# Christina-hshi/SH-assembly

Hardware: AMD Instinct MI355X
Metric: k-mers counted/sec (whole node), CQF build, C.elegans-like k=47 (higher is better)
Workload: dtype u64

## Files before the change

### sh-assembly_amd/csrc/partition_kernels.hip

```cpp
#include "shk_device.h"

#define SHK_RP_TILE 4096
#define SHK_RP_MAXP 1024
#define SHK_SCAN_TILE 2048

struct ShkRpLevel {
  uint32_t shift;
  uint32_t bits;
  uint32_t nbuckets;
  uint32_t hb;
  uint64_t q_lo;
  uint64_t nslots;
  uint32_t out32;
  uint32_t ablate;
  uint32_t slot_cap;
  uint32_t ng_log2;
};

__device__ __forceinline__ uint32_t shk_word_region(uint64_t w, uint32_t hb, uint64_t q_lo) {
  uint64_t key = hb >= 64 ? w : (w & ((1ULL << hb) - 1));
  return (uint32_t)(((key >> 8) - q_lo) >> SHK_REGION_LOG2);
}

template <typename T>
__global__ void k_scan_reduce(const T *in, uint64_t n_host, const uint64_t *n_dev, uint64_t *block_sums) {
  __shared__ uint64_t scratch[SHK_MAX_WAVES + 1];
  const uint64_t n = n_dev ? *n_dev : n_host;
  const uint64_t base = (uint64_t)blockIdx.x * SHK_SCAN_TILE;
  uint64_t s = 0;
  for (uint64_t i = base + threadIdx.x; i < base + SHK_SCAN_TILE && i < n; i += blockDim.x) s += in[i];
  uint64_t tot = shk_block_sum64(s, scratch);
  if (threadIdx.x == 0) block_sums[blockIdx.x] = tot;
}
__global__ void k_scan_top(uint64_t *block_sums, uint64_t nblocks, uint64_t *total) {
  __shared__ uint64_t scratch[SHK_MAX_WAVES + 1];
  __shared__ uint64_t carry_s;
  if (threadIdx.x == 0) carry_s = 0;
  __syncthreads();
  for (uint64_t b = 0; b < nblocks; b += blockDim.x) {
    uint64_t i = b + threadIdx.x;
    uint64_t v = i < nblocks ? block_sums[i] : 0, tot;
    uint64_t ex = shk_block_exscan64(v, &tot, scratch);
    uint64_t carry = carry_s;
    if (i < nblocks) block_sums[i] = carry + ex;
    __syncthreads();
    if (threadIdx.x == 0) carry_s = carry + tot;
    __syncthreads();
  }
  if (threadIdx.x == 0) *total = carry_s;
}
template <typename T>
__global__ void k_scan_apply(const T *in, uint64_t n_host, const uint64_t *n_dev, const uint64_t *block_sums,
                             const uint64_t *total, uint64_t *out) {
  __shared__ uint64_t scratch[SHK_MAX_WAVES + 1];
  const uint64_t n = n_dev ? *n_dev : n_host;
  const uint64_t base = (uint64_t)blockIdx.x * SHK_SCAN_TILE;
  if (base > n) return;
  const unsigned per = SHK_SCAN_TILE / blockDim.x;
  const uint64_t my = base + (uint64_t)threadIdx.x * per;
  uint64_t s = 0;
  for (unsigned j = 0; j < per; j++)
    if (my + j < n) s += in[my + j];
  uint64_t tot;
  uint64_t ex = shk_block_exscan64(s, &tot, scratch) + block_sums[blockIdx.x];
  for (unsigned j = 0; j < per; j++) {
    if (my + j < n) { out[my + j] = ex; ex += in[my + j]; }
  }
  if (threadIdx.x == 0 && n >= base && n < base + SHK_SCAN_TILE) out[n] = *total;
}

__global__ void k_rp_base1(const uint64_t *n_p, uint64_t *bucket_base) {
  if (threadIdx.x == 0 && blockIdx.x == 0) { bucket_base[0] = 0; bucket_base[1] = *n_p; }
}

__global__ void k_rp_tile_first(const uint64_t *bucket_base, uint32_t nbuckets, const uint64_t *n_p, uint32_t *tfb) {
  const uint64_t n = *n_p;
  const uint64_t w = (uint64_t)blockIdx.x * blockDim.x + threadIdx.x;
  const uint64_t pos = w * SHK_RP_TILE;
  if (pos >= n) return;
  uint32_t lo = 0, hi = nbuckets;
  while (hi - lo > 1) {
    uint32_t mid = (lo + hi) / 2;
    if (bucket_base[mid] <= pos) lo = mid; else hi = mid;
  }
  tfb[w] = lo;
}

__global__ void k_rp_hist(const uint64_t *words, const uint64_t *n_p, const uint64_t *bucket_base,
                          const uint32_t *tfb, ShkRpLevel lv, uint64_t *hist, uint32_t wtiles) {
  __shared__ uint32_t lh[SHK_RP_MAXP];
  const uint64_t n = *n_p;
  const uint64_t wstart = (uint64_t)blockIdx.x * wtiles * SHK_RP_TILE;
  if (wstart >= n) return;
  const uint64_t wend = wstart + (uint64_t)wtiles * SHK_RP_TILE < n ? wstart + (uint64_t)wtiles * SHK_RP_TILE : n;
  const uint32_t P = 1u << lv.bits;
  for (uint32_t b = tfb[(uint64_t)blockIdx.x * wtiles]; b < lv.nbuckets && bucket_base[b] < wend; b++) {
    const uint64_t lo = bucket_base[b] > wstart ? bucket_base[b] : wstart;
    const uint64_t hi = bucket_base[b + 1] < wend ? bucket_base[b + 1] : wend;
    if (hi <= lo) continue;
    for (uint32_t d = threadIdx.x; d < (P << lv.ng_log2); d += blockDim.x) lh[d] = 0;
    __syncthreads();
    for (uint64_t i0 = lo; i0 < hi; i0 += 4ull * blockDim.x) {
      uint64_t w[4];
#pragma unroll
      for (int u = 0; u < 4; u++) {
        const uint64_t i = i0 + (uint64_t)u * blockDim.x + threadIdx.x;
        w[u] = i < hi ? words[i] : 0;
      }
#pragma unroll
      for (int u = 0; u < 4; u++) {
        const uint64_t i = i0 + (uint64_t)u * blockDim.x + threadIdx.x;
        if (i < hi) {
          const uint32_t dg = (shk_word_region(w[u], lv.hb, lv.q_lo) >> lv.shift) & (P - 1);
          const uint32_t grp = (uint32_t)(i >> SHK_RP_TILE0_LOG2) & ((1u << lv.ng_log2) - 1);
          atomicAdd(&lh[(dg << lv.ng_log2) | grp], 1u);
        }
      }
    }
    __syncthreads();
    for (uint32_t d = threadIdx.x; d < (P << lv.ng_log2); d += blockDim.x)
      if (lh[d]) atomicAdd((unsigned long long *)&hist[(((uint64_t)b * P) << lv.ng_log2) + d], (unsigned long long)lh[d]);
    __syncthreads();
  }
}

__global__ void k_rp_group_bases(const uint64_t *sub, uint32_t nd, uint32_t ng_log2, uint64_t *base) {
  const uint32_t d = blockIdx.x * blockDim.x + threadIdx.x;
  if (d <= nd) base[d] = sub[(uint64_t)d << ng_log2];
}

#define SHK_RP_THREADS 512
#define SHK_RP_KPT (SHK_RP_TILE / SHK_RP_THREADS)
template <int LB2>
__global__ void k_rp_hist2(const uint64_t *words, const uint64_t *n_p, ShkRpLevel lv0, ShkRpLevel lv1, uint64_t *hist0, uint64_t *hist1,
                           uint32_t wtiles) {
  __shared__ uint32_t lh0[SHK_RP_MAXP];
  __shared__ uint32_t lh1[1u << LB2];
  const uint64_t n = *n_p;
  const uint64_t wstart = (uint64_t)blockIdx.x * wtiles * SHK_RP_TILE;
  if (wstart >= n) return;
  const uint64_t wend = wstart + (uint64_t)wtiles * SHK_RP_TILE < n ? wstart + (uint64_t)wtiles * SHK_RP_TILE : n;
  const uint32_t P0 = 1u << lv0.bits, C = 1u << (lv0.bits + lv1.bits);
  for (uint32_t d = threadIdx.x; d < (P0 << lv0.ng_log2); d += blockDim.x) lh0[d] = 0;
  for (uint32_t d = threadIdx.x; d < C; d += blockDim.x) lh1[d] = 0;
  __syncthreads();
  for (uint64_t i0 = wstart; i0 < wend; i0 += 4ull * blockDim.x) {
    uint64_t w[4];
#pragma unroll
    for (int u = 0; u < 4; u++) {
      const uint64_t i = i0 + (uint64_t)u * blockDim.x + threadIdx.x;
      w[u] = i < wend ? words[i] : 0;
    }
#pragma unroll
    for (int u = 0; u < 4; u++) {
      const uint64_t i = i0 + (uint64_t)u * blockDim.x + threadIdx.x;
      if (i < wend) {
        const uint32_t region = shk_word_region(w[u], lv0.hb, lv0.q_lo);
        const uint32_t d0 = (region >> lv0.shift) & (P0 - 1);
        const uint32_t grp = (uint32_t)(i >> SHK_RP_TILE0_LOG2) & ((1u << lv0.ng_log2) - 1);
        atomicAdd(&lh0[(d0 << lv0.ng_log2) | grp], 1u);
        atomicAdd(&lh1[(region >> lv1.shift) & (C - 1)], 1u);
      }
    }
  }
  __syncthreads();
  for (uint32_t d = threadIdx.x; d < (P0 << lv0.ng_log2); d += blockDim.x)
    if (lh0[d]) atomicAdd((unsigned long long *)&hist0[d], (unsigned long long)lh0[d]);
  for (uint32_t d = threadIdx.x; d < C; d += blockDim.x)
    if (lh1[d]) atomicAdd((unsigned long long *)&hist1[d], (unsigned long long)lh1[d]);
}

__global__ void k_rp_slot_cursors(uint64_t *cursor, uint64_t n, uint32_t cap) {
  const uint64_t stride = (uint64_t)gridDim.x * blockDim.x;
  for (uint64_t i = (uint64_t)blockIdx.x * blockDim.x + threadIdx.x; i < n; i += stride) cursor[i] = i * cap;
}

template <int TILE_LOG2, int THREADS, int PMAX = SHK_RP_MAXP>
__global__ void __launch_bounds__(THREADS) k_rp_scatter(const uint64_t *in, uint64_t *out, const uint64_t *n_p,
                                                        const uint64_t *bucket_base, const uint32_t *tfb, ShkRpLevel lv,
                                                        uint64_t *cursor, uint32_t *err) {
  constexpr uint32_t SHK_RP_TILE_ = 1u << TILE_LOG2;
  constexpr int KPT_ = (int)(SHK_RP_TILE_ / THREADS);
  static_assert(SHK_RP_TILE_ <= 65536, "a rank inside a digit takes 16 bits");
  __shared__ uint32_t lh[PMAX];
  __shared__ uint32_t lbase[PMAX];
  __shared__ uint64_t gbase[PMAX];
  __shared__ uint64_t stage[SHK_RP_TILE_];
  __shared__ uint32_t scratch[SHK_MAX_WAVES + 1];
  const uint64_t n = *n_p;
  const uint64_t wstart = (uint64_t)blockIdx.x * SHK_RP_TILE_;
  if (wstart >= n) return;
  const uint64_t wend = wstart + SHK_RP_TILE_ < n ? wstart + SHK_RP_TILE_ : n;
  const uint32_t P = 1u << lv.bits;
  for (uint32_t b = (lv.nbuckets > 1 ? tfb[(uint64_t)blockIdx.x << (TILE_LOG2 - 12)] : 0u); b < lv.nbuckets && bucket_base[b] < wend; b++) {
    const uint64_t lo = bucket_base[b] > wstart ? bucket_base[b] : wstart;
    const uint64_t hi = bucket_base[b + 1] < wend ? bucket_base[b + 1] : wend;
    if (hi <= lo) continue;
    const uint32_t cnt = (uint32_t)(hi - lo);
    for (uint32_t d = threadIdx.x; d < P; d += THREADS) lh[d] = 0;
    uint64_t w[KPT_];
#pragma unroll
    for (int u = 0; u < KPT_; u++) {
      const uint32_t i = threadIdx.x + (uint32_t)u * THREADS;
      w[u] = i < cnt ? in[lo + i] : 0;
    }
    __syncthreads();
    uint32_t dr[KPT_];
#pragma unroll
    for (int u = 0; u < KPT_; u++) {
      const uint32_t i = threadIdx.x + (uint32_t)u * THREADS;
      dr[u] = 0;
      if (i < cnt) {
        const uint32_t d = (shk_word_region(w[u], lv.hb, lv.q_lo) >> lv.shift) & (P - 1);
        dr[u] = (d << 16) | atomicAdd(&lh[d], 1u);
      }
    }
    __syncthreads();
    uint32_t carry = 0;
    for (uint32_t d0 = 0; d0 < P; d0 += THREADS) {
      uint32_t d = d0 + threadIdx.x;
      uint32_t v = d < P ? lh[d] : 0, tot;
      uint32_t ex = shk_block_exscan(v, &tot, scratch);
      if (d < P) {
        lbase[d] = carry + ex;
        if (lv.ablate & 1) gbase[d] = cursor[((uint64_t)b * P + d) << lv.ng_log2] + (uint64_t)(blockIdx.x % 1024) * 24;
        else gbase[d] = v ? atomicAdd((unsigned long long *)&cursor[((((uint64_t)b * P) + d) << lv.ng_log2) | (blockIdx.x & ((1u << lv.ng_log2) - 1))], (unsigned long long)v) : 0;
        if (lv.slot_cap && v && gbase[d] + v > ((uint64_t)b * P + d + 1) * lv.slot_cap) {
          atomicOr(err, SHK_E_SLOT_FULL);
          gbase[d] = ~0ULL;
        }
      }
      carry += tot;
    }
    __syncthreads();
#pragma unroll
    for (int u = 0; u < KPT_; u++) {
      const uint32_t i = threadIdx.x + (uint32_t)u * THREADS;
      if (i < cnt) stage[lbase[dr[u] >> 16] + (dr[u] & 0xFFFFu)] = w[u];
    }
    __syncthreads();
    for (uint32_t i = threadIdx.x; i < cnt; i += THREADS) {
      uint64_t x = stage[i];
      uint32_t d = (shk_word_region(x, lv.hb, lv.q_lo) >> lv.shift) & (P - 1);
      if (lv.out32) {
        const uint64_t key = lv.hb >= 64 ? x : (x & ((1ULL << lv.hb) - 1));
        const uint64_t q = (key >> 8) - lv.q_lo;
        if (q >= lv.nslots) atomicOr(err, SHK_E_CORRUPT);
        const uint32_t rec = ((((uint32_t)q & (SHK_REGION - 1)) << 8 | (uint32_t)(key & 0xff)) << SHK_CHUNK_BITS) |
                             ((uint32_t)(x >> lv.hb) & (SHK_MAX_CHUNKS - 1));
        if (gbase[d] != ~0ULL) reinterpret_cast<uint32_t *>(out)[gbase[d] + (i - lbase[d])] = rec;
      } else {
        out[gbase[d] + (i - lbase[d])] = x;
      }
    }
    shk_lds_barrier();
  }
}
```

### sh-assembly_amd/csrc/shk_api.hip

```cpp
#include "../../include/shk.h"
#include <thread>

#include <hip/hip_runtime.h>
#include <math.h>
#include <stdio.h>
#include <stdlib.h>
#include <string.h>
#include <vector>
#include <string>
#include <algorithm>
#include <unordered_set>
#include <unordered_map>

#include "kmer_kernels.hip"
#include "roll_kernels.hip"
#include "partition_kernels.hip"
#include "cqf_kernels.hip"
#include "merge2_kernels.hip"
#include "walk_kernels.hip"
#include "unitig_kernels.hip"

#define SHK_SLACK 256

enum {
  KP_COUNT_LINES, KP_SCAN_CHUNKS, KP_EMIT_READS, KP_COUNT_KEYS, KP_HASH, KP_SCAN, KP_RP_PREP, KP_RP_HIST,
  KP_RP_SCATTER, KP_MERGE_SUM, KP_REGION_SCAN, KP_MERGE_WRITE, KP_MERGE_SPILL, KP_PLACE, KP_MARKS, KP_LOOKUP, KP_WALK, KP_UG_WALK, KP_UG_FINISH, KP_MERGE_FUSED, KP_MERGE_SAMPLE, KP_MISC, KP_ROLL_HIST, KP_ROLL_SCATTER, KP_PACK, KP_RP_SLOTS, KP_N
};
static const char *kp_names[KP_N] = {
  "k_count_lines", "k_scan_chunks", "k_emit_reads", "k_count_keys", "k_hash_reads", "k_scan_*", "k_rp_prep",
  "k_rp_hist", "k_rp_scatter", "k_region_merge<summary>", "k_region_scan", "k_region_merge<write>",
  "k_region_merge<spill>", "k_region_place", "k_denoise_marks", "k_lookup", "k_extend_forward+k_select_seeds", "k_ug_walk", "k_ug_check/emit/median/links", "k_region_merge<fused>", "k_region_merge<sample>", "misc", "k_roll_hist", "k_roll_scatter", "k_pack_reads", "k_rp_slot_cursors"};

struct PendingEvent { int id; hipEvent_t a, b; };

#define SHK_SCALAR_WORDS 64
enum ShkDevSlot {
  DS_NREADS = 0,
  DS_NWORDS = 1,
  DS_SCAN_TOTAL = 2,
  DS_MARKS = 3,
  DS_MAX_COUNT = 4,
  DS_DUMP_STOP = 5,
  DS_WALK_IN = 8,
  DS_WALK_OUT = 10,
  DS_STAMPS = 16,
  DS_PAIR_LEN = 40,
  DS_PAIR_BASE = 42,
  DS_END = 46
};
enum ShkHostSlot {
  HP_COUNTERS = 0,
  HP_ERR = 40,
  HP_NREADS = 41,
  HP_NWORDS = 42,
  HP_NWORDS_IN = 43,
  HP_FREE_PTR = 44,
  HP_TOTAL = 45,
  HP_AUX = 46,
  HP_MARKS = 47,
  HP_IFIN = 48,
  HP_IFIRST = 49,
  HP_WALK_IN = 50,
  HP_WALK_OUT = 52,
  HP_PAIR = 56,
  HP_END = 62
};
enum { CNT_NEWD, CNT_ADDED, CNT_REMOVED, CNT_ADDED_BEFORE };
static_assert(HP_COUNTERS + SHK_NCOUNTERS <= HP_ERR, "the counters mirror ends before the error word");
static_assert(DS_END <= SHK_SCALAR_WORDS && HP_END <= SHK_SCALAR_WORDS, "both blocks fit their 64 words");
static_assert(DS_PAIR_BASE + 4 == DS_END && HP_PAIR + (DS_END - DS_PAIR_LEN) == HP_END, "the pair block is uploaded in one copy");

enum { RP_SCATTER_GROUPED, RP_SCATTER_WIDE, RP_SCATTER_TILE };
struct ShkPartLevel {
  uint8_t scatter;
  bool pair_hist;
  bool may_slot;
};

struct ShkStageBufs {
  hipStream_t stream = hipStream_t();
  bool lent = false;
  uint8_t *d_text = nullptr;
  uint64_t *d_chunk_off = nullptr, *d_chunk_len = nullptr, *d_nlines = nullptr, *d_reads_base = nullptr;
  uint64_t *d_rd_start = nullptr, *d_rd_end = nullptr;
  uint16_t *d_rd_chunk = nullptr;
  uint32_t *d_nkeys = nullptr;
  uint64_t *d_key_base = nullptr;
  uint64_t *d_words[2] = {};
  uint64_t *d_scalars = nullptr;
  uint64_t *d_block_sums = nullptr;
  uint64_t *d_hist[4] = {};
  uint64_t *d_base_sub = nullptr;
  uint64_t *d_base[5] = {};
  uint64_t *d_cursor = nullptr;
  uint32_t *d_tfb = nullptr;
  uint32_t *d_err = nullptr;
  uint64_t *h_pinned = nullptr;
  uint32_t last_err_bits = 0;
  uint32_t region_cap = 0;
  uint32_t slot_overflows = 0;
  int slots_off = 0;
  double prof_ms[KP_N] = {};
  uint64_t prof_n[KP_N] = {};
  std::vector<PendingEvent> pending;
  std::vector<hipEvent_t> evpool;
};

struct shk_ctx : ShkStageBufs {
  shk_config cfg;
// ... 161 lines not shown
  for (uint32_t l = 0; l < 4; l++) hipFree(b->d_hist[l]);
  for (uint32_t l = 0; l < 5; l++) if (!(b->lent && l == c->nlevels)) hipFree(b->d_base[l]);
  hipHostFree(b->h_pinned);
  if (b->stream) hipStreamDestroy(b->stream);
  *b = ShkStageBufs();
}

static int create_init(shk_ctx *c, const shk_config *cfg) {
  const uint32_t ns = cfg->num_shards ? cfg->num_shards : 1;
  c->cfg = *cfg;
  c->dev = cfg->device;
  HIPCHK(hipSetDevice(c->dev));
  c->g_nslots = 1ULL << cfg->qb;
  if (c->g_nslots / ns < 64) return SHK_ERR_ARG;
  c->nslots = c->g_nslots / ns;
  c->q_lo = c->nslots * cfg->shard_index;
  c->xnslots = c->nslots + (uint64_t)(10 * sqrt((double)c->g_nslots));
  c->nblocks = (c->xnslots + 63) / 64;
  c->table_bytes = c->nblocks * SHK_BLOCK_BYTES;
  c->nregions = (uint32_t)((c->nslots + SHK_REGION - 1) / SHK_REGION);
  c->rbits = 0;
  while ((1u << c->rbits) < c->nregions) c->rbits++;
  const uint32_t mlb = cfg->max_level_bits ? cfg->max_level_bits : 10;
  if (mlb > 10) return SHK_ERR_ARG;
  const uint32_t nlevels = (c->rbits + mlb - 1) / mlb;
  if (nlevels > 4) return SHK_ERR_ARG;
  c->nlevels = nlevels ? nlevels : 1;
  {
    uint32_t left = c->rbits, nb = 1;
    for (uint32_t l = 0; l < c->nlevels; l++) {
      uint32_t bits = (left + (c->nlevels - l) - 1) / (c->nlevels - l);
      left -= bits;
      c->lv[l].shift = left; c->lv[l].bits = bits; c->lv[l].nbuckets = nb; c->lv[l].hb = cfg->hb; c->lv[l].q_lo = c->q_lo;
      c->lv[l].nslots = c->nslots; c->lv[l].out32 = 0; c->lv[l].ablate = 0; c->lv[l].ng_log2 = 0; c->lv[l].slot_cap = 0;
      nb <<= bits;
    }
    c->lv[c->nlevels - 1].out32 = 1;
    if (c->lv[0].bits >= 2 && c->lv[0].bits <= 7 && !getenv("SHK_RP_NO_GROUPS")) c->lv[0].ng_log2 = 3;
  }
  c->threads = cfg->threads_per_group ? cfg->threads_per_group : 512;
  if (c->threads < 64 || c->threads > 1024 || (c->threads & (c->threads - 1))) return SHK_ERR_ARG;
  c->hash_groups = cfg->hash_groups ? cfg->hash_groups : 2048;
  c->roll_two = c->nlevels >= 2 && c->lv[0].bits + c->lv[1].bits <= 14;
  for (uint32_t l = 0; l < c->nlevels; l++) {
    const bool last = l + 1 == c->nlevels;
    c->part[l].scatter = l == 0 && c->lv[0].ng_log2 ? RP_SCATTER_GROUPED : c->threads >= 512 && !last && c->lv[l].bits <= 8 ? RP_SCATTER_WIDE : RP_SCATTER_TILE;
    c->part[l].pair_hist = l == 0 && c->roll_two && c->lv[1].ng_log2 == 0;
    c->part[l].may_slot = last && l >= 1 && c->lv[l].out32;
  }
  c->rounds_left = cfg->num_denoise;
  c->max_reads = cfg->max_batch_reads ? cfg->max_batch_reads : cfg->max_batch_bytes / 16 + 1024;
  { int rc = bufs_alloc(c, c, false); if (rc) return rc; }
  for (int i = 0; i < 2; i++) {
    if (dmalloc(&c->tab[i], c->table_bytes)) return SHK_ERR_HIP;
    if (dmalloc(&c->fin[i], (uint64_t)c->nregions + 2)) return SHK_ERR_HIP;
  }
  if (dmalloc(&c->d_summary, SHK_SUM_STRIDE * (uint64_t)c->nregions + 8)) return SHK_ERR_HIP;
  if (dmalloc(&c->d_dump_offs, (uint64_t)c->nregions + 2)) return SHK_ERR_HIP;
  c->sample_stride = c->nregions >= (1u << 20) ? 16 : 8;
  if (const char *e = getenv("SHK_SAMPLE_STRIDE")) c->sample_stride = (uint32_t)atoi(e);
  else if (c->nregions < (1u << 14)) c->sample_stride = 0;
  c->lazy_ok = 1;
  if (const char *e = getenv("SHK_LAZY_PLACE")) c->lazy_ok = atoi(e) != 0;
  if (dmalloc(&c->spill[0], (uint64_t)c->nregions * SHK_SPILL_STRIDE) || dmalloc(&c->d_over_list, (uint64_t)c->nregions + 1)) return SHK_ERR_HIP;
  { uint64_t nt = c->nregions / SHK_RSCAN_TILE + 2;
    if (dmalloc(&c->d_tile_a, nt) || dmalloc(&c->d_tile_b, nt) || dmalloc(&c->d_tile_f, nt)) return SHK_ERR_HIP; }
  if (dmalloc(&c->d_counters, SHK_NCOUNTERS)) return SHK_ERR_HIP;
  HIPCHK(hipMemsetAsync(c->tab[0], 0, c->table_bytes + SHK_SLACK, c->stream));
  HIPCHK(hipMemsetAsync(c->tab[1], 0, c->table_bytes + SHK_SLACK, c->stream));
  HIPCHK(hipMemsetAsync(c->fin[0], 0, ((uint64_t)c->nregions + 2) * 8, c->stream));
  HIPCHK(hipMemsetAsync(c->fin[1], 0, ((uint64_t)c->nregions + 2) * 8, c->stream));
  HIPCHK(hipStreamSynchronize(c->stream));
  if (cfg->num_denoise > 0 || cfg->num_shards > 1) {
    if (ensure_chist(c) || point_alloc(c)) return SHK_ERR_HIP;
  }
  if (cfg->num_shards > 1) {
    for (int b = 0; b < 2; b++)
      if (dmalloc(&c->d_send[b], c->cfg.max_batch_keys + 1)) return SHK_ERR_HIP;
  }
  return SHK_OK;
}
// ... 188 lines not shown
  if (!chunk_labels_ok(nchunks, chunk_first, chunk_mul)) return SHK_ERR_BATCH;
  const uint8_t *dtext;
  uint64_t nreads;
  { int rc = parse_stage(c, b, text, on_device, text_bytes, chunk_off, chunk_len, nchunks, &dtext, &nreads); if (rc) return rc; }
  const uint64_t P = 1ULL << c->lv[0].bits;
  const uint32_t cb = c->lv[0].bits + c->lv[1].bits;
  const bool two = c->roll_two;
  if (two) HIPCHK(hipMemsetAsync(b->d_hist[1], 0, (1ULL << cb) * 8, b->stream));
  else HIPCHK(hipMemsetAsync(b->d_hist[0], 0, P * 8, b->stream));
  ShkRollArgs A;
  roll_args(c, b, A, dtext, text_bytes, chunk_first, chunk_mul);
  A.q_lo = c->q_lo;
  A.dig_shift = c->lv[0].shift; A.dig_bits = c->lv[0].bits;
  A.hist = two ? b->d_hist[1] : b->d_hist[0]; A.hist_shift = two ? c->lv[1].shift : c->lv[0].shift; A.hist_bits = two ? cb : c->lv[0].bits;
  A.cursor = b->d_cursor; A.out = b->d_words[0];
  { int rc = pack_stage(c, b, A, nreads, text_bytes, b->d_words[1]); if (rc) return rc; }
  { ProfScope ps(c, b, KP_ROLL_HIST);
    launch_roll_hist(c, b, A, nreads, two);
    if (two) hipLaunchKernelGGL(k_roll_fold, dim3((uint32_t)(P / 256 + 1)), dim3(256), 0, b->stream, (const uint64_t *)b->d_hist[1], (uint32_t)P,
                                1u << c->lv[1].bits, b->d_hist[0]); }
  if (run_scan<uint64_t>(c, b, b->d_hist[0], P, nullptr, b->d_base[1])) return SHK_ERR_HIP;
  HIPCHK(hipMemcpyAsync(b->d_scalars + DS_NWORDS, b->d_base[1] + P, 8, hipMemcpyDeviceToDevice, b->stream));
  HIPCHK(hipMemcpyAsync(b->d_cursor, b->d_base[1], P * 8, hipMemcpyDeviceToDevice, b->stream));
  launch_roll_scatter(c, b, A, nreads);
  HIPCHK(hipGetLastError());
  return SHK_OK;
}

struct ShkPartInput {
  const uint64_t *src[2]; uint64_t n[2]; int nsrc;
  int in_buf;
  uint32_t first_level;
  bool counted[2];
};
static ShkPartInput part_from_roll(const shk_ctx *c, const ShkStageBufs *b, uint64_t n) { return {{b->d_words[0], nullptr}, {n, 0}, 1, 0, 1, {false, c->roll_two}}; }
static ShkPartInput part_from_hash(const ShkStageBufs *b, uint64_t n) { return {{b->d_words[0], nullptr}, {n, 0}, 1, 0, 0, {true, false}}; }
static ShkPartInput part_from_words(const ShkStageBufs *b, const uint64_t *w, uint64_t n, const uint64_t *w2 = nullptr, uint64_t n2 = 0) {
  return {{w, w2}, {n, n2}, w2 ? 2 : 1, w == b->d_words[0] ? 0 : w == b->d_words[1] ? 1 : -1, 0, {false, false}};
}

static uint32_t slot_capacity(const shk_ctx *c, uint64_t nregions, uint64_t nwords) {
  uint64_t cp = 2 * c->cfg.max_batch_keys / nregions;
  if (cp > (1u << 20)) cp = 1u << 20;
  const double mean = (double)nwords / (double)nregions;
  return cp >= 64 && (double)cp >= mean + 6.0 * sqrt(8.0 * mean + 1.0) + 16.0 ? (uint32_t)cp : 0;
}

static int partition_stage(const shk_ctx *c, ShkStageBufs *b, const ShkPartInput &in, int *dst) {
  const uint64_t *n_p = b->d_scalars + DS_NWORDS;
  const uint64_t nmax = in.n[0] + in.n[1];
  { ProfScope ps(c, b, KP_RP_PREP);
    hipLaunchKernelGGL(k_rp_base1, dim3(1), dim3(64), 0, b->stream, n_p, b->d_base[0]); }
  const uint32_t nwin = (uint32_t)(nmax / SHK_RP_TILE + 1);
  int cur = in.in_buf < 0 ? 1 : in.in_buf;
  bool counted[4] = {in.counted[0], in.counted[1], false, false};
  b->region_cap = 0;
  for (uint32_t l = in.first_level; l < c->nlevels; l++) {
    const ShkPartLevel &pl = c->part[l];
    const uint64_t nb = c->lv[l].nbuckets, P = 1ULL << c->lv[l].bits;
    struct Src { const uint64_t *w, *n_p, *base; uint64_t n; } srcs[2] = {{l == in.first_level ? in.src[0] : b->d_words[cur], n_p, b->d_base[l], nmax}, {}};
    int nsrc = 1;
    if (l == 0 && in.nsrc == 2) {
      srcs[0] = {in.src[0], b->d_scalars + DS_PAIR_LEN, b->d_scalars + DS_PAIR_BASE, in.n[0]};
      srcs[1] = {in.src[1], b->d_scalars + DS_PAIR_LEN + 1, b->d_scalars + DS_PAIR_BASE + 2, in.n[1]};
      nsrc = 2;
    }
    uint32_t cap = pl.may_slot && !b->slots_off && !counted[l] ? slot_capacity(c, nb * P, nmax) : 0;
    { ProfScope ps(c, b, KP_RP_PREP);
      hipLaunchKernelGGL(k_rp_tile_first, dim3(nwin / 256 + 1), dim3(256), 0, b->stream, b->d_base[l], (uint32_t)nb, n_p, b->d_tfb); }
    for (;;) {
      ShkRpLevel lvl = c->lv[l];
#ifdef SHK_DIAGNOSTICS
      if (const char *e = getenv("SHK_RP_ABLATE")) lvl.ablate = (uint32_t)atoi(e);
#endif
      uint64_t *cursor = b->d_cursor;
      if (cap) {
        ProfScope ps(c, b, KP_RP_SLOTS);
        cursor = b->d_base[l + 1];
        lvl.slot_cap = cap;
        hipLaunchKernelGGL(k_rp_slot_cursors, dim3((uint32_t)((nb * P) / 256 + 1 < 4096 ? (nb * P) / 256 + 1 : 4096)), dim3(256), 0, b->stream, cursor, nb * P, cap);
      } else {
        if (!counted[l] && pl.pair_hist) {
          HIPCHK(hipMemsetAsync(b->d_hist[0], 0, (P << c->lv[0].ng_log2) * 8, b->stream));
          HIPCHK(hipMemsetAsync(b->d_hist[1], 0, (P << c->lv[1].bits) * 8, b->stream));
          ProfScope ps(c, b, KP_RP_HIST);
          const uint32_t wt = nwin / 1024 + 1;
          for (int si = 0; si < nsrc; si++)
            hipLaunchKernelGGL((k_rp_hist2<14>), dim3(nwin / wt + 1), dim3(c->threads < 512 ? c->threads : 512), 0, b->stream, srcs[si].w, srcs[si].n_p,
                               c->lv[0], c->lv[1], b->d_hist[0], b->d_hist[1], wt);
          counted[1] = true;
        } else if (!counted[l]) {
          HIPCHK(hipMemsetAsync(b->d_hist[l], 0, ((nb * P) << c->lv[l].ng_log2) * 8, b->stream));
          ProfScope ps(c, b, KP_RP_HIST);
          const uint32_t wt = nwin / 4096 + 1;
          for (int si = 0; si < nsrc; si++)
            hipLaunchKernelGGL(k_rp_hist, dim3(nwin / wt + 1), dim3(c->threads), 0, b->stream, srcs[si].w, srcs[si].n_p, srcs[si].base, b->d_tfb, c->lv[l],
                               b->d_hist[l], wt);
        }
        if (c->lv[l].ng_log2) {
          const uint32_t ng = c->lv[l].ng_log2;
          if (run_scan<uint64_t>(c, b, b->d_hist[l], P << ng, nullptr, b->d_base_sub)) return SHK_ERR_HIP;
          HIPCHK(hipMemcpyAsync(b->d_cursor, b->d_base_sub, (P << ng) * 8, hipMemcpyDeviceToDevice, b->stream));
          ProfScope ps(c, b, KP_RP_PREP);
          hipLaunchKernelGGL(k_rp_group_bases, dim3((uint32_t)(P / 256 + 1)), dim3(256), 0, b->stream, b->d_base_sub, (uint32_t)P, ng, b->d_base[l + 1]);
        } else {
          if (run_scan<uint64_t>(c, b, b->d_hist[l], nb * P, nullptr, b->d_base[l + 1])) return SHK_ERR_HIP;
          HIPCHK(hipMemcpyAsync(b->d_cursor, b->d_base[l + 1], nb * P * 8, hipMemcpyDeviceToDevice, b->stream));
        }
      }
      { ProfScope ps(c, b, KP_RP_SCATTER);
        for (int si = 0; si < nsrc; si++) {
          const Src &S = srcs[si];
          const dim3 wide((uint32_t)(S.n >> SHK_RP_TILE0_LOG2) + 1);
          if (pl.scatter == RP_SCATTER_GROUPED)
            hipLaunchKernelGGL((k_rp_scatter<SHK_RP_TILE0_LOG2, 1024>), wide, dim3(1024), 0, b->stream, S.w, b->d_words[cur ^ 1], S.n_p, S.base,
                               b->d_tfb, lvl, cursor, b->d_err);
          else if (pl.scatter == RP_SCATTER_WIDE)
            hipLaunchKernelGGL((k_rp_scatter<SHK_RP_TILE0_LOG2, 1024, 256>), wide, dim3(1024), 0, b->stream, S.w, b->d_words[cur ^ 1], S.n_p, S.base,
                               b->d_tfb, lvl, cursor, b->d_err);
          else
            hipLaunchKernelGGL((k_rp_scatter<12, SHK_RP_THREADS>), dim3((uint32_t)(S.n / SHK_RP_TILE + 1)), dim3(SHK_RP_THREADS), 0, b->stream, S.w,
                               b->d_words[cur ^ 1], S.n_p, S.base, b->d_tfb, lvl, cursor, b->d_err);
        } }
      if (!cap) break;
      uint32_t bits = 0;
      if (fetch_err(b, &bits)) return SHK_ERR_HIP;
      if (bits & ~SHK_E_SLOT_FULL) return map_err_bits(bits & ~SHK_E_SLOT_FULL);
      if (!bits) { b->region_cap = cap; b->slot_overflows = 0; break; }
      if (++b->slot_overflows >= 2) b->slots_off = 1;
      cap = 0;
    }
    cur ^= 1;
  }
  HIPCHK(hipGetLastError());
  *dst = cur;
  return SHK_OK;
}

#define SHK_REGION_SLICE (1u << 24)
#define SHK_FOR_REGION_SLICES(c, A, nblk) \
  for (uint32_t r0_ = 0, nblk = 0; r0_ < (c)->nregions && ((A).r0 = r0_, nblk = (c)->nregions - r0_ < SHK_REGION_SLICE ? (c)->nregions - r0_ : SHK_REGION_SLICE, true); r0_ += SHK_REGION_SLICE)

template <int MODE>
static void launch_merge(shk_ctx *c, const ShkMergeArgs &A0, bool rec = false) {
  ShkMergeArgs A = A0;
  SHK_FOR_REGION_SLICES(c, A, nblk) {
    if (MODE != 1 && rec)
// ... 550 lines not shown

static int merge_stage(shk_ctx *c, const uint64_t *words, uint32_t nchunks, uint64_t nwords, shk_batch_stats *st) {
  uint32_t lo = 0;
  int rc = merge_stage_from(c, words, nchunks, nwords, st, &lo);
  if (rc == SHK_ERR_REGION && !c->big_image && (c->last_err_bits & (SHK_E_OLD_EXTENT | SHK_E_NEW_EXTENT))) {
    c->big_image = 1;
    c->last_err_bits = 0;
    rc = merge_stage_from(c, words, nchunks, nwords, st, &lo);
  }
  return rc;
}

static int finish(shk_ctx *c, int rc) {
  uint32_t bits = 0;
  int rc2 = fetch_err(c, &bits);
  prof_collect(c);
  if (rc) return rc;
  if (rc2) return rc2;
  return map_err_bits(bits);
}

static int front_end(const shk_ctx *c, ShkStageBufs *b, const void *text, int on_device, uint64_t text_bytes, const uint64_t *chunk_off,
                     const uint64_t *chunk_len, uint32_t nchunks, uint64_t *nwords, int *dst, uint32_t *region_cap) {
  const bool roll = roll_path(c);
  int rc = roll ? roll_stage(c, b, text, on_device, text_bytes, chunk_off, chunk_len, nchunks, 0, 1)
                : hash_stage(c, b, text, on_device, text_bytes, chunk_off, chunk_len, nchunks, 0, 1, true);
  if (rc) return rc;
  uint32_t bits = 0;
  HIPCHK(hipMemcpyAsync(b->h_pinned + HP_NWORDS, b->d_scalars + DS_NWORDS, 8, hipMemcpyDeviceToHost, b->stream));
  if (fetch_err(b, &bits)) return SHK_ERR_HIP;
  if (bits) return map_err_bits(bits);
  *nwords = b->h_pinned[HP_NWORDS];
  if (*nwords > c->cfg.max_batch_keys) return SHK_ERR_BATCH;
  rc = partition_stage(c, b, roll ? part_from_roll(c, b, *nwords) : part_from_hash(b, *nwords), dst);
  *region_cap = b->region_cap;
  return rc;
}

extern "C" int shk_count_chunks(shk_ctx *c, const void *text, int text_on_device, uint64_t text_bytes,
                                const uint64_t *chunk_off, const uint64_t *chunk_len, uint32_t nchunks,
                                shk_batch_stats *stats) {
  if (!c || !text || !chunk_off || !chunk_len) return SHK_ERR_ARG;
  shk_batch_stats st;
  memset(&st, 0, sizeof(st));
  HIPCHK(hipSetDevice(c->dev));
  if (upload_wait(c, text, text_on_device, c->stream)) return SHK_ERR_HIP;
  uint64_t nwords = 0;
  int dst = 0;
  uint32_t cap = 0;
  int rc = front_end(c, c, text, text_on_device, text_bytes, chunk_off, chunk_len, nchunks, &nwords, &dst, &cap);
  if (rc) return finish(c, rc);
  rc = merge_stage(c, c->d_words[dst], nchunks, nwords, &st);
  if (stats) *stats = st;
  return finish(c, rc);
}

struct ShkFrontSlot {
  uint64_t *words = nullptr;
  uint64_t *base = nullptr;
  uint32_t cap = 0;
  std::thread th;
  bool busy = false;
  int rc = 0;
  uint64_t nwords = 0;
  uint32_t nchunks = 0;
};
struct ShkFront {
// ... 182 lines not shown
template <typename F>
static int owner_bins(shk_ctx *c, uint32_t nbins, uint32_t per_owner, F count, uint64_t *counts, std::vector<uint64_t> &base) {
  uint64_t *hist = c->d_block_sums + ROUTE_HIST;
  HIPCHK(hipMemsetAsync(hist, 0, nbins * 8, c->stream));
  count();
  std::vector<uint64_t> hh(nbins);
  HIPCHK(hipMemcpyAsync(hh.data(), hist, nbins * 8, hipMemcpyDeviceToHost, c->stream));
  uint32_t bits = 0;
  if (fetch_err(c, &bits)) return SHK_ERR_HIP;
  if (bits) return map_err_bits(bits);
  base.assign(nbins + 1, 0);
  std::fill(counts, counts + nbins / per_owner, 0);
  for (uint32_t i = 0; i < nbins; i++) { counts[i / per_owner] += hh[i]; base[i + 1] = base[i] + hh[i]; }
  HIPCHK(hipMemcpyAsync(c->d_block_sums + ROUTE_CURSOR, base.data(), nbins * 8, hipMemcpyHostToDevice, c->stream));
  return SHK_OK;
}

extern "C" int shk_route_words(shk_ctx *c, uint64_t nwords, uint32_t nshards, uint64_t **d_out, uint64_t *counts) {
  if (!c || !d_out || !counts || nshards == 0 || (nshards & (nshards - 1)) || nshards > SHK_RP_MAXP) return SHK_ERR_ARG;
  if (nwords > c->cfg.max_batch_keys) return SHK_ERR_BATCH;
  HIPCHK(hipSetDevice(c->dev));
  uint32_t lg = 0;
  while ((1u << lg) < nshards) lg++;
  uint64_t *send;
  if (send_buffer(c, &send)) return SHK_ERR_HIP;
  if (lg == 0) {
    HIPCHK(hipMemcpyAsync(send, c->d_words[0], nwords * 8, hipMemcpyDeviceToDevice, c->stream));
    *d_out = send; counts[0] = nwords;
    return finish(c, 0);
  }
  if (c->cfg.qb < SHK_REGION_LOG2 + lg) return SHK_ERR_ARG;
  ShkRpLevel lv;
  lv.shift = (c->cfg.qb - SHK_REGION_LOG2) - lg; lv.bits = lg; lv.nbuckets = 1; lv.hb = c->cfg.hb; lv.q_lo = 0;
  lv.nslots = ~0ULL; lv.out32 = 0; lv.ablate = 0; lv.ng_log2 = 0; lv.slot_cap = 0;
  if (set_nwords(c, nwords)) return SHK_ERR_HIP;
  const uint64_t *n_p = c->d_scalars + DS_NWORDS;
  const uint32_t nwin = (uint32_t)(nwords / SHK_RP_TILE + 1);
  { ProfScope ps(c, KP_RP_PREP);
    hipLaunchKernelGGL(k_rp_base1, dim3(1), dim3(64), 0, c->stream, n_p, c->d_base[0]);
    hipLaunchKernelGGL(k_rp_tile_first, dim3(nwin / 256 + 1), dim3(256), 0, c->stream, c->d_base[0], 1u, n_p, c->d_tfb); }
  std::vector<uint64_t> base;
  int rc = owner_bins(c, nshards, 1, [&] {
    ProfScope ps(c, KP_RP_HIST);
    const uint32_t wt = nwin / 4096 + 1;
    hipLaunchKernelGGL(k_rp_hist, dim3(nwin / wt + 1), dim3(c->threads), 0, c->stream, c->d_words[0], n_p, c->d_base[0], c->d_tfb, lv, c->d_block_sums + ROUTE_HIST, wt);
  }, counts, base);
  if (rc) return finish(c, rc);
  { ProfScope ps(c, KP_RP_SCATTER);
    hipLaunchKernelGGL((k_rp_scatter<12, SHK_RP_THREADS>), dim3(nwin), dim3(SHK_RP_THREADS), 0, c->stream, c->d_words[0], send, n_p,
                       c->d_base[0], c->d_tfb, lv, c->d_block_sums + ROUTE_CURSOR, c->d_err); }
  HIPCHK(hipGetLastError());
  *d_out = send;
  return finish(c, 0);
}

extern "C" int shk_hash_route_chunks(shk_ctx *c, const void *text, int text_on_device, uint64_t text_bytes, const uint64_t *chunk_off,
                                     const uint64_t *chunk_len, uint32_t nchunks, uint32_t nshards, uint64_t **d_out, uint64_t *counts,
                                     uint64_t *nwords) {
  if (!c || !text || !chunk_off || !chunk_len || !d_out || !counts || !nwords) return SHK_ERR_ARG;
  if (nshards == 0 || (nshards & (nshards - 1)) || nshards > SHK_RP_MAXP) return SHK_ERR_ARG;
  HIPCHK(hipSetDevice(c->dev));
  uint32_t lg = 0;
  while ((1u << lg) < nshards) lg++;
  if (c->cfg.qb < SHK_REGION_LOG2 + lg) return SHK_ERR_ARG;
  const uint32_t chunk_first = c->cfg.shard_index, chunk_mul = c->cfg.num_shards ? c->cfg.num_shards : 1;
  if (!chunk_labels_ok(nchunks, chunk_first, chunk_mul)) return SHK_ERR_BATCH;
  uint64_t *send;
  if (send_buffer(c, &send)) return SHK_ERR_HIP;
  const uint8_t *dtext;
  uint64_t nreads;
  if (upload_wait(c, text, text_on_device, c->stream)) return SHK_ERR_HIP;
  int rc = parse_stage(c, c, text, text_on_device, text_bytes, chunk_off, chunk_len, nchunks, &dtext, &nreads);
  if (rc) return finish(c, rc);
  const uint32_t rb = c->cfg.qb - SHK_REGION_LOG2;
  const uint32_t db = lg > 7 ? lg : (rb < 7 ? (rb > lg ? rb : lg) : 7);
  const uint32_t nbins = 1u << db, per_owner = nbins / nshards;
  ShkRollArgs A;
  roll_args(c, c, A, dtext, text_bytes, chunk_first, chunk_mul);
// ... 1143 lines not shown
```

Before: 33.40 billion.

## Narrow radix-partition records to 32 bits one level before the last

At the second-to-last partition level, the scatter now packs each 64-bit word into a 32-bit record holding the remaining region bits, the low key byte and the chunk id, and writes it out. The last level's histogram and scatter then read these 32-bit records directly. This halves the read and write traffic of the final partition pass and shrinks its LDS staging buffer. The narrow path only applies when the chunk count fits in the available chunk bits, and an environment variable can turn it off. It adds new code paths whose bit layout must match the existing final-record format.

```diff
diff --git a/sh-assembly_amd/csrc/partition_kernels.hip b/sh-assembly_amd/csrc/partition_kernels.hip
--- a/sh-assembly_amd/csrc/partition_kernels.hip
+++ b/sh-assembly_amd/csrc/partition_kernels.hip
@@ -1,4 +1,5 @@
 #include "shk_device.h"
+#include <type_traits>
 
 #define SHK_RP_TILE 4096
 #define SHK_RP_MAXP 1024
@@ -11,6 +12,7 @@
   uint32_t hb;
   uint64_t q_lo;
   uint64_t nslots;
+  uint32_t cb;
   uint32_t out32;
   uint32_t ablate;
   uint32_t slot_cap;
@@ -20,6 +22,13 @@
 __device__ __forceinline__ uint32_t shk_word_region(uint64_t w, uint32_t hb, uint64_t q_lo) {
   uint64_t key = hb >= 64 ? w : (w & ((1ULL << hb) - 1));
   return (uint32_t)(((key >> 8) - q_lo) >> SHK_REGION_LOG2);
+}
+
+enum { RP_WORDS = 0, RP_NARROW_OUT = 1, RP_NARROW_IN = 2 };
+__device__ __forceinline__ uint32_t shk_narrow_rec(uint64_t w, uint32_t hb, uint64_t q_lo, uint32_t cb) {
+  const uint64_t key = hb >= 64 ? w : (w & ((1ULL << hb) - 1));
+  const uint32_t up = (uint32_t)(key - (q_lo << 8)) & ((1u << (32 - cb)) - 1);
+  return (up << cb) | ((uint32_t)(w >> hb) & ((1u << cb) - 1));
 }
 
 template <typename T>
@@ -86,9 +95,12 @@
   tfb[w] = lo;
 }
 
-__global__ void k_rp_hist(const uint64_t *words, const uint64_t *n_p, const uint64_t *bucket_base,
+template <bool NARROW>
+__global__ void k_rp_hist(const uint64_t *words_, const uint64_t *n_p, const uint64_t *bucket_base,
                           const uint32_t *tfb, ShkRpLevel lv, uint64_t *hist, uint32_t wtiles) {
   __shared__ uint32_t lh[SHK_RP_MAXP];
+  using W = typename std::conditional<NARROW, uint32_t, uint64_t>::type;
+  const W *words = reinterpret_cast<const W *>(words_);
   const uint64_t n = *n_p;
   const uint64_t wstart = (uint64_t)blockIdx.x * wtiles * SHK_RP_TILE;
   if (wstart >= n) return;
@@ -101,7 +113,7 @@
     for (uint32_t d = threadIdx.x; d < (P << lv.ng_log2); d += blockDim.x) lh[d] = 0;
     __syncthreads();
     for (uint64_t i0 = lo; i0 < hi; i0 += 4ull * blockDim.x) {
-      uint64_t w[4];
+      W w[4];
 #pragma unroll
       for (int u = 0; u < 4; u++) {
         const uint64_t i = i0 + (uint64_t)u * blockDim.x + threadIdx.x;
@@ -111,7 +123,7 @@
       for (int u = 0; u < 4; u++) {
         const uint64_t i = i0 + (uint64_t)u * blockDim.x + threadIdx.x;
         if (i < hi) {
-          const uint32_t dg = (shk_word_region(w[u], lv.hb, lv.q_lo) >> lv.shift) & (P - 1);
+          const uint32_t dg = NARROW ? (uint32_t)(w[u] >> (16 + lv.cb)) : (shk_word_region(w[u], lv.hb, lv.q_lo) >> lv.shift) & (P - 1);
           const uint32_t grp = (uint32_t)(i >> SHK_RP_TILE0_LOG2) & ((1u << lv.ng_log2) - 1);
           atomicAdd(&lh[(dg << lv.ng_log2) | grp], 1u);
         }
@@ -175,17 +187,20 @@
   for (uint64_t i = (uint64_t)blockIdx.x * blockDim.x + threadIdx.x; i < n; i += stride) cursor[i] = i * cap;
 }
 
-template <int TILE_LOG2, int THREADS, int PMAX = SHK_RP_MAXP>
-__global__ void __launch_bounds__(THREADS) k_rp_scatter(const uint64_t *in, uint64_t *out, const uint64_t *n_p,
+template <int TILE_LOG2, int THREADS, int PMAX = SHK_RP_MAXP, int FORM = RP_WORDS>
+__global__ void __launch_bounds__(THREADS) k_rp_scatter(const uint64_t *in_, uint64_t *out, const uint64_t *n_p,
                                                         const uint64_t *bucket_base, const uint32_t *tfb, ShkRpLevel lv,
                                                         uint64_t *cursor, uint32_t *err) {
   constexpr uint32_t SHK_RP_TILE_ = 1u << TILE_LOG2;
   constexpr int KPT_ = (int)(SHK_RP_TILE_ / THREADS);
   static_assert(SHK_RP_TILE_ <= 65536, "a rank inside a digit takes 16 bits");
+  using WIN = typename std::conditional<FORM == RP_NARROW_IN, uint32_t, uint64_t>::type;
+  using WST = typename std::conditional<FORM == RP_WORDS, uint64_t, uint32_t>::type;
+  const WIN *in = reinterpret_cast<const WIN *>(in_);
   __shared__ uint32_t lh[PMAX];
   __shared__ uint32_t lbase[PMAX];
   __shared__ uint64_t gbase[PMAX];
-  __shared__ uint64_t stage[SHK_RP_TILE_];
+  __shared__ WST stage[SHK_RP_TILE_];
   __shared__ uint32_t scratch[SHK_MAX_WAVES + 1];
   const uint64_t n = *n_p;
   const uint64_t wstart = (uint64_t)blockIdx.x * SHK_RP_TILE_;
@@ -198,7 +213,7 @@
     if (hi <= lo) continue;
     const uint32_t cnt = (uint32_t)(hi - lo);
     for (uint32_t d = threadIdx.x; d < P; d += THREADS) lh[d] = 0;
-    uint64_t w[KPT_];
+    WIN w[KPT_];
 #pragma unroll
     for (int u = 0; u < KPT_; u++) {
       const uint32_t i = threadIdx.x + (uint32_t)u * THREADS;
@@ -206,12 +221,21 @@
     }
     __syncthreads();
     uint32_t dr[KPT_];
+    WST x[KPT_];
 #pragma unroll
     for (int u = 0; u < KPT_; u++) {
       const uint32_t i = threadIdx.x + (uint32_t)u * THREADS;
       dr[u] = 0;
+      x[u] = (WST)w[u];
       if (i < cnt) {
-        const uint32_t d = (shk_word_region(w[u], lv.hb, lv.q_lo) >> lv.shift) & (P - 1);
+        uint32_t d;
+        if (FORM == RP_NARROW_IN) d = (uint32_t)(w[u] >> (16 + lv.cb));
+        else d = (shk_word_region(w[u], lv.hb, lv.q_lo) >> lv.shift) & (P - 1);
+        if (FORM == RP_NARROW_OUT) {
+          const uint64_t key = lv.hb >= 64 ? w[u] : (w[u] & ((1ULL << lv.hb) - 1));
+          if ((key >> 8) - lv.q_lo >= lv.nslots) atomicOr(err, SHK_E_CORRUPT);
+          x[u] = (WST)shk_narrow_rec(w[u], lv.hb, lv.q_lo, lv.cb);
+        }
         dr[u] = (d << 16) | atomicAdd(&lh[d], 1u);
       }
     }
@@ -236,21 +260,37 @@
 #pragma unroll
     for (int u = 0; u < KPT_; u++) {
       const uint32_t i = threadIdx.x + (uint32_t)u * THREADS;
-      if (i < cnt) stage[lbase[dr[u] >> 16] + (dr[u] & 0xFFFFu)] = w[u];
-    }
-    __syncthreads();
-    for (uint32_t i = threadIdx.x; i < cnt; i += THREADS) {
-      uint64_t x = stage[i];
-      uint32_t d = (shk_word_region(x, lv.hb, lv.q_lo) >> lv.shift) & (P - 1);
-      if (lv.out32) {
-        const uint64_t key = lv.hb >= 64 ? x : (x & ((1ULL << lv.hb) - 1));
-        const uint64_t q = (key >> 8) - lv.q_lo;
-        if (q >= lv.nslots) atomicOr(err, SHK_E_CORRUPT);
-        const uint32_t rec = ((((uint32_t)q & (SHK_REGION - 1)) << 8 | (uint32_t)(key & 0xff)) << SHK_CHUNK_BITS) |
-                             ((uint32_t)(x >> lv.hb) & (SHK_MAX_CHUNKS - 1));
-        if (gbase[d] != ~0ULL) reinterpret_cast<uint32_t *>(out)[gbase[d] + (i - lbase[d])] = rec;
-      } else {
-        out[gbase[d] + (i - lbase[d])] = x;
+      if (i < cnt) stage[lbase[dr[u] >> 16] + (dr[u] & 0xFFFFu)] = x[u];
+    }
+    __syncthreads();
+    if (FORM == RP_NARROW_OUT) {
+      uint32_t *out32 = reinterpret_cast<uint32_t *>(out);
+      for (uint32_t d = threadIdx.x / SHK_WAVE; d < P; d += THREADS / SHK_WAVE) {
+        const uint32_t l0 = lbase[d], len = lh[d];
+        const uint64_t g0 = gbase[d];
+        for (uint32_t j = threadIdx.x % SHK_WAVE; j < len; j += SHK_WAVE) out32[g0 + j] = stage[l0 + j];
+      }
+    } else {
+      for (uint32_t i = threadIdx.x; i < cnt; i += THREADS) {
+        const WST xs = stage[i];
+        if (FORM == RP_NARROW_IN) {
+          const uint32_t d = xs >> (16 + lv.cb);
+          const uint32_t rec = (((uint32_t)(xs >> lv.cb) & 0xFFFFu) << SHK_CHUNK_BITS) | ((uint32_t)xs & ((1u << lv.cb) - 1));
+          if (gbase[d] != ~0ULL) reinterpret_cast<uint32_t *>(out)[gbase[d] + (i - lbase[d])] = rec;
+          continue;
+        }
+        const uint64_t x64 = xs;
+        uint32_t d = (shk_word_region(x64, lv.hb, lv.q_lo) >> lv.shift) & (P - 1);
+        if (lv.out32) {
+          const uint64_t key = lv.hb >= 64 ? x64 : (x64 & ((1ULL << lv.hb) - 1));
+          const uint64_t q = (key >> 8) - lv.q_lo;
+          if (q >= lv.nslots) atomicOr(err, SHK_E_CORRUPT);
+          const uint32_t rec = ((((uint32_t)q & (SHK_REGION - 1)) << 8 | (uint32_t)(key & 0xff)) << SHK_CHUNK_BITS) |
+                               ((uint32_t)(x64 >> lv.hb) & (SHK_MAX_CHUNKS - 1));
+          if (gbase[d] != ~0ULL) reinterpret_cast<uint32_t *>(out)[gbase[d] + (i - lbase[d])] = rec;
+        } else {
+          out[gbase[d] + (i - lbase[d])] = x64;
+        }
       }
     }
     shk_lds_barrier();
diff --git a/sh-assembly_amd/csrc/shk_api.hip b/sh-assembly_amd/csrc/shk_api.hip
--- a/sh-assembly_amd/csrc/shk_api.hip
+++ b/sh-assembly_amd/csrc/shk_api.hip
@@ -24,12 +24,12 @@
 
 enum {
   KP_COUNT_LINES, KP_SCAN_CHUNKS, KP_EMIT_READS, KP_COUNT_KEYS, KP_HASH, KP_SCAN, KP_RP_PREP, KP_RP_HIST,
-  KP_RP_SCATTER, KP_MERGE_SUM, KP_REGION_SCAN, KP_MERGE_WRITE, KP_MERGE_SPILL, KP_PLACE, KP_MARKS, KP_LOOKUP, KP_WALK, KP_UG_WALK, KP_UG_FINISH, KP_MERGE_FUSED, KP_MERGE_SAMPLE, KP_MISC, KP_ROLL_HIST, KP_ROLL_SCATTER, KP_PACK, KP_RP_SLOTS, KP_N
+  KP_RP_SCATTER, KP_MERGE_SUM, KP_REGION_SCAN, KP_MERGE_WRITE, KP_MERGE_SPILL, KP_PLACE, KP_MARKS, KP_LOOKUP, KP_WALK, KP_UG_WALK, KP_UG_FINISH, KP_MERGE_FUSED, KP_MERGE_SAMPLE, KP_MISC, KP_ROLL_HIST, KP_ROLL_SCATTER, KP_PACK, KP_RP_SLOTS, KP_RP_SCATTER_NARROW, KP_N
 };
 static const char *kp_names[KP_N] = {
   "k_count_lines", "k_scan_chunks", "k_emit_reads", "k_count_keys", "k_hash_reads", "k_scan_*", "k_rp_prep",
   "k_rp_hist", "k_rp_scatter", "k_region_merge<summary>", "k_region_scan", "k_region_merge<write>",
-  "k_region_merge<spill>", "k_region_place", "k_denoise_marks", "k_lookup", "k_extend_forward+k_select_seeds", "k_ug_walk", "k_ug_check/emit/median/links", "k_region_merge<fused>", "k_region_merge<sample>", "misc", "k_roll_hist", "k_roll_scatter", "k_pack_reads", "k_rp_slot_cursors"};
+  "k_region_merge<spill>", "k_region_place", "k_denoise_marks", "k_lookup", "k_extend_forward+k_select_seeds", "k_ug_walk", "k_ug_check/emit/median/links", "k_region_merge<fused>", "k_region_merge<sample>", "misc", "k_roll_hist", "k_roll_scatter", "k_pack_reads", "k_rp_slot_cursors", "k_rp_scatter<narrow>"};
 
 struct PendingEvent { int id; hipEvent_t a, b; };
 
@@ -75,6 +75,7 @@
   uint8_t scatter;
   bool pair_hist;
   bool may_slot;
+  bool may_narrow;
 };
 
 struct ShkStageBufs {
@@ -302,7 +303,7 @@
       uint32_t bits = (left + (c->nlevels - l) - 1) / (c->nlevels - l);
       left -= bits;
       c->lv[l].shift = left; c->lv[l].bits = bits; c->lv[l].nbuckets = nb; c->lv[l].hb = cfg->hb; c->lv[l].q_lo = c->q_lo;
-      c->lv[l].nslots = c->nslots; c->lv[l].out32 = 0; c->lv[l].ablate = 0; c->lv[l].ng_log2 = 0; c->lv[l].slot_cap = 0;
+      c->lv[l].nslots = c->nslots; c->lv[l].cb = 0; c->lv[l].out32 = 0; c->lv[l].ablate = 0; c->lv[l].ng_log2 = 0; c->lv[l].slot_cap = 0;
       nb <<= bits;
     }
     c->lv[c->nlevels - 1].out32 = 1;
@@ -311,12 +312,15 @@
   c->threads = cfg->threads_per_group ? cfg->threads_per_group : 512;
   if (c->threads < 64 || c->threads > 1024 || (c->threads & (c->threads - 1))) return SHK_ERR_ARG;
   c->hash_groups = cfg->hash_groups ? cfg->hash_groups : 2048;
+  const bool words8 = getenv("SHK_RP_WORDS8") && atoi(getenv("SHK_RP_WORDS8")) != 0;
   c->roll_two = c->nlevels >= 2 && c->lv[0].bits + c->lv[1].bits <= 14;
   for (uint32_t l = 0; l < c->nlevels; l++) {
     const bool last = l + 1 == c->nlevels;
     c->part[l].scatter = l == 0 && c->lv[0].ng_log2 ? RP_SCATTER_GROUPED : c->threads >= 512 && !last && c->lv[l].bits <= 8 ? RP_SCATTER_WIDE : RP_SCATTER_TILE;
     c->part[l].pair_hist = l == 0 && c->roll_two && c->lv[1].ng_log2 == 0;
     c->part[l].may_slot = last && l >= 1 && c->lv[l].out32;
+    c->part[l].may_narrow = l >= 1 && l + 2 == c->nlevels && !words8;
+    c->lv[l].cb = 32 - 16 - c->lv[c->nlevels - 1].bits;
   }
   c->rounds_left = cfg->num_denoise;
   c->max_reads = cfg->max_batch_reads ? cfg->max_batch_reads : cfg->max_batch_bytes / 16 + 1024;
@@ -571,11 +575,12 @@
   int in_buf;
   uint32_t first_level;
   bool counted[2];
+  uint32_t nchunks;
 };
-static ShkPartInput part_from_roll(const shk_ctx *c, const ShkStageBufs *b, uint64_t n) { return {{b->d_words[0], nullptr}, {n, 0}, 1, 0, 1, {false, c->roll_two}}; }
-static ShkPartInput part_from_hash(const ShkStageBufs *b, uint64_t n) { return {{b->d_words[0], nullptr}, {n, 0}, 1, 0, 0, {true, false}}; }
+static ShkPartInput part_from_roll(const shk_ctx *c, const ShkStageBufs *b, uint64_t n, uint32_t nchunks) { return {{b->d_words[0], nullptr}, {n, 0}, 1, 0, 1, {false, c->roll_two}, nchunks}; }
+static ShkPartInput part_from_hash(const ShkStageBufs *b, uint64_t n, uint32_t nchunks) { return {{b->d_words[0], nullptr}, {n, 0}, 1, 0, 0, {true, false}, nchunks}; }
 static ShkPartInput part_from_words(const ShkStageBufs *b, const uint64_t *w, uint64_t n, const uint64_t *w2 = nullptr, uint64_t n2 = 0) {
-  return {{w, w2}, {n, n2}, w2 ? 2 : 1, w == b->d_words[0] ? 0 : w == b->d_words[1] ? 1 : -1, 0, {false, false}};
+  return {{w, w2}, {n, n2}, w2 ? 2 : 1, w == b->d_words[0] ? 0 : w == b->d_words[1] ? 1 : -1, 0, {false, false}, 0};
 }
 
 static uint32_t slot_capacity(const shk_ctx *c, uint64_t nregions, uint64_t nwords) {
@@ -593,10 +598,13 @@
   const uint32_t nwin = (uint32_t)(nmax / SHK_RP_TILE + 1);
   int cur = in.in_buf < 0 ? 1 : in.in_buf;
   bool counted[4] = {in.counted[0], in.counted[1], false, false};
+  bool narrow = false;
   b->region_cap = 0;
   for (uint32_t l = in.first_level; l < c->nlevels; l++) {
     const ShkPartLevel &pl = c->part[l];
     const uint64_t nb = c->lv[l].nbuckets, P = 1ULL << c->lv[l].bits;
+    const bool narrow_in = narrow;
+    narrow = pl.may_narrow && in.nchunks && in.nchunks <= (1u << c->lv[l].cb);
     struct Src { const uint64_t *w, *n_p, *base; uint64_t n; } srcs[2] = {{l == in.first_level ? in.src[0] : b->d_words[cur], n_p, b->d_base[l], nmax}, {}};
     int nsrc = 1;
     if (l == 0 && in.nsrc == 2) {
@@ -633,8 +641,12 @@
           ProfScope ps(c, b, KP_RP_HIST);
           const uint32_t wt = nwin / 4096 + 1;
           for (int si = 0; si < nsrc; si++)
-            hipLaunchKernelGGL(k_rp_hist, dim3(nwin / wt + 1), dim3(c->threads), 0, b->stream, srcs[si].w, srcs[si].n_p, srcs[si].base, b->d_tfb, c->lv[l],
-                               b->d_hist[l], wt);
+            if (narrow_in)
+              hipLaunchKernelGGL(k_rp_hist<true>, dim3(nwin / wt + 1), dim3(c->threads), 0, b->stream, srcs[si].w, srcs[si].n_p, srcs[si].base, b->d_tfb,
+                                 c->lv[l], b->d_hist[l], wt);
+            else
+              hipLaunchKernelGGL(k_rp_hist<false>, dim3(nwin / wt + 1), dim3(c->threads), 0, b->stream, srcs[si].w, srcs[si].n_p, srcs[si].base, b->d_tfb,
+                                 c->lv[l], b->d_hist[l], wt);
         }
         if (c->lv[l].ng_log2) {
           const uint32_t ng = c->lv[l].ng_log2;
@@ -647,11 +659,20 @@
           HIPCHK(hipMemcpyAsync(b->d_cursor, b->d_base[l + 1], nb * P * 8, hipMemcpyDeviceToDevice, b->stream));
         }
       }
-      { ProfScope ps(c, b, KP_RP_SCATTER);
+      { ProfScope ps(c, b, narrow || narrow_in ? KP_RP_SCATTER_NARROW : KP_RP_SCATTER);
         for (int si = 0; si < nsrc; si++) {
           const Src &S = srcs[si];
           const dim3 wide((uint32_t)(S.n >> SHK_RP_TILE0_LOG2) + 1);
-          if (pl.scatter == RP_SCATTER_GROUPED)
+          if (narrow && pl.scatter == RP_SCATTER_WIDE)
+            hipLaunchKernelGGL((k_rp_scatter<SHK_RP_TILE0_LOG2, 1024, 256, RP_NARROW_OUT>), wide, dim3(1024), 0, b->stream, S.w, b->d_words[cur ^ 1], S.n_p,
+                               S.base, b->d_tfb, lvl, cursor, b->d_err);
+          else if (narrow)
+            hipLaunchKernelGGL((k_rp_scatter<12, SHK_RP_THREADS, SHK_RP_MAXP, RP_NARROW_OUT>), dim3((uint32_t)(S.n / SHK_RP_TILE + 1)), dim3(SHK_RP_THREADS), 0,
+                               b->stream, S.w, b->d_words[cur ^ 1], S.n_p, S.base, b->d_tfb, lvl, cursor, b->d_err);
+          else if (narrow_in)
+            hipLaunchKernelGGL((k_rp_scatter<12, SHK_RP_THREADS, SHK_RP_MAXP, RP_NARROW_IN>), dim3((uint32_t)(S.n / SHK_RP_TILE + 1)), dim3(SHK_RP_THREADS), 0,
+                               b->stream, S.w, b->d_words[cur ^ 1], S.n_p, S.base, b->d_tfb, lvl, cursor, b->d_err);
+          else if (pl.scatter == RP_SCATTER_GROUPED)
             hipLaunchKernelGGL((k_rp_scatter<SHK_RP_TILE0_LOG2, 1024>), wide, dim3(1024), 0, b->stream, S.w, b->d_words[cur ^ 1], S.n_p, S.base,
                                b->d_tfb, lvl, cursor, b->d_err);
           else if (pl.scatter == RP_SCATTER_WIDE)
@@ -1268,7 +1289,7 @@
   if (bits) return map_err_bits(bits);
   *nwords = b->h_pinned[HP_NWORDS];
   if (*nwords > c->cfg.max_batch_keys) return SHK_ERR_BATCH;
-  rc = partition_stage(c, b, roll ? part_from_roll(c, b, *nwords) : part_from_hash(b, *nwords), dst);
+  rc = partition_stage(c, b, roll ? part_from_roll(c, b, *nwords, nchunks) : part_from_hash(b, *nwords, nchunks), dst);
   *region_cap = b->region_cap;
   return rc;
 }
@@ -1517,7 +1538,7 @@
   if (c->cfg.qb < SHK_REGION_LOG2 + lg) return SHK_ERR_ARG;
   ShkRpLevel lv;
   lv.shift = (c->cfg.qb - SHK_REGION_LOG2) - lg; lv.bits = lg; lv.nbuckets = 1; lv.hb = c->cfg.hb; lv.q_lo = 0;
-  lv.nslots = ~0ULL; lv.out32 = 0; lv.ablate = 0; lv.ng_log2 = 0; lv.slot_cap = 0;
+  lv.nslots = ~0ULL; lv.cb = 0; lv.out32 = 0; lv.ablate = 0; lv.ng_log2 = 0; lv.slot_cap = 0;
   if (set_nwords(c, nwords)) return SHK_ERR_HIP;
   const uint64_t *n_p = c->d_scalars + DS_NWORDS;
   const uint32_t nwin = (uint32_t)(nwords / SHK_RP_TILE + 1);
@@ -1528,7 +1549,7 @@
   int rc = owner_bins(c, nshards, 1, [&] {
     ProfScope ps(c, KP_RP_HIST);
     const uint32_t wt = nwin / 4096 + 1;
-    hipLaunchKernelGGL(k_rp_hist, dim3(nwin / wt + 1), dim3(c->threads), 0, c->stream, c->d_words[0], n_p, c->d_base[0], c->d_tfb, lv, c->d_block_sums + ROUTE_HIST, wt);
+    hipLaunchKernelGGL(k_rp_hist<false>, dim3(nwin / wt + 1), dim3(c->threads), 0, c->stream, c->d_words[0], n_p, c->d_base[0], c->d_tfb, lv, c->d_block_sums + ROUTE_HIST, wt);
   }, counts, base);
   if (rc) return finish(c, rc);
   { ProfScope ps(c, KP_RP_SCATTER);
```

After: 34.59 billion (median of 6 runs). +3.6%, better.
